# mikelodder7/bls-bn254

Hardware: AMD Instinct MI355X
Metric: BN254 pairings/sec (= BLS verifies/sec) (higher is better)
Workload: dtype int64; 1 GPU; 262144 batched single-sig BLS verifies per GPU (BASELINE configs[1]), unique 32-byte messages, 1024-key pool, 1/64 invalid tuples; key de-duplication + hash-to-G1 + per-key G2 checks and line tables + 2-pair Miller loop + final exp; tuples_per_gpu=262144, tuples_total=262144, key_pool=1024

## Files before the change

### bls-bn254_amd/csrc/host.hip

```cpp
#include "host_common.h"

extern "C" {

const uint8_t NEG_G2_BYTES[128] = {
  0x19,0x8e,0x93,0x93,0x92,0x0d,0x48,0x3a,0x72,0x60,0xbf,0xb7,0x31,0xfb,0x5d,0x25,0xf1,0xaa,0x49,0x33,0x35,0xa9,0xe7,0x12,0x97,0xe4,0x85,0xb7,0xae,0xf3,0x12,0xc2,
  0x18,0x00,0xde,0xef,0x12,0x1f,0x1e,0x76,0x42,0x6a,0x00,0x66,0x5e,0x5c,0x44,0x79,0x67,0x43,0x22,0xd4,0xf7,0x5e,0xda,0xdd,0x46,0xde,0xbd,0x5c,0xd9,0x92,0xf6,0xed,
  0x27,0x5d,0xc4,0xa2,0x88,0xd1,0xaf,0xb3,0xcb,0xb1,0xac,0x09,0x18,0x75,0x24,0xc7,0xdb,0x36,0x39,0x5d,0xf7,0xbe,0x3b,0x99,0xe6,0x73,0xb1,0x3a,0x07,0x5a,0x65,0xec,
  0x1d,0x9b,0xef,0xcd,0x05,0xa5,0x32,0x3e,0x6d,0xa4,0xd4,0x35,0xf3,0xb6,0x17,0xcd,0xb3,0xaf,0x83,0x28,0x5c,0x2d,0xf7,0x11,0xef,0x39,0xc0,0x15,0x71,0x82,0x7f,0x9d};


const char* blsbn254_strerror(int code) {
  switch (code) {
    case 0: return "ok";
    case 1: return "invalid scalar bytes";
    case 2: return "invalid G1 bytes";
    case 3: return "invalid G2 bytes";
    case 4: return "invalid Gt bytes";
    case BLSBN254_ST_SHORT: return "too few usable partial signatures";
    case BLSBN254_E_ARG: return "invalid argument";
    case BLSBN254_E_HIP: return "HIP runtime error";
    case BLSBN254_E_NOMEM: return "out of device memory";
    case BLSBN254_E_NO_DEVICE: return "no gfx950 device available (there is no CPU fallback)";
    case BLSBN254_E_RCCL: return "RCCL error";
    default: return "unknown error";
  }
}
const char* blsbn254_last_error(blsbn254_ctx* ctx) { return ctx ? ctx->last_error.c_str() : ""; }

int blsbn254_ctx_create(int device, blsbn254_ctx** out) {
  if (!out) return BLSBN254_E_ARG;
  *out = nullptr;
  int count = 0;
  if (hipGetDeviceCount(&count) != hipSuccess || count <= 0 || device < 0 || device >= count) return BLSBN254_E_NO_DEVICE;
  hipDeviceProp_t prop;
  if (hipGetDeviceProperties(&prop, device) != hipSuccess) return BLSBN254_E_NO_DEVICE;
  if (std::strncmp(prop.gcnArchName, "gfx950", 6) != 0) return BLSBN254_E_NO_DEVICE;
  blsbn254_ctx* c = new blsbn254_ctx();
  c->device = device;
  if (const char* e = std::getenv("BLSBN254_CHUNK_LANES")) {
    size_t v = (size_t)std::strtoull(e, nullptr, 10) & ~(size_t)7;
    if (v >= 8 && v <= ((size_t)1 << 23)) c->chunk = v;
  }
  if (hipSetDevice(device) != hipSuccess || hipStreamCreateWithFlags(&c->stream, hipStreamNonBlocking) != hipSuccess) { delete c; return BLSBN254_E_HIP; }
  if (hipStreamCreateWithFlags(&c->stream2, hipStreamNonBlocking) != hipSuccess || hipEventCreateWithFlags(&c->ev_fork, hipEventDisableTiming) != hipSuccess ||
      hipEventCreateWithFlags(&c->ev_join, hipEventDisableTiming) != hipSuccess) { (void)hipStreamDestroy(c->stream); delete c; return BLSBN254_E_HIP; }
  if (getrandom(&c->kd_seed, sizeof c->kd_seed, 0) != (ssize_t)sizeof c->kd_seed) c->kd_seed = 0x5bd1e995u;
  if (const char* e = std::getenv("BLSBN254_AUTO_PREPARE")) c->auto_prepare = std::atoi(e) != 0;
  if (const char* e = std::getenv("BLSBN254_RLC_GROUP")) { long v = std::atol(e); if (v >= 2 && v <= 4096) { c->rlc_group = (size_t)v; c->rlc_group_auto = false; } }
  c->lanes_per_round = (size_t)prop.multiProcessorCount * 256;
  if (const char* e = std::getenv("BLSBN254_RLC_KEY_ROUND")) c->rlc_key_round = std::atoi(e) != 0;
  if (const char* e = std::getenv("BLSBN254_WIDE_FE")) c->wide_fe = std::atoi(e) != 0;
  if (const char* e = std::getenv("BLSBN254_ASYNC_VERIFY")) c->async_verify = std::atoi(e) != 0;
  if (const char* e = std::getenv("BLSBN254_KEY_CACHE")) { long v = std::atol(e); if (v >= 0 && v <= (long)PREP_MAX_KEYS) c->kc.max = (size_t)v; }
  if (const char* e = std::getenv("BLSBN254_QUAD_PREP")) c->quad_prep = std::atoi(e) != 0;
  if (const char* e = std::getenv("BLSBN254_SPLIT_EASY")) c->split_easy = std::atoi(e) != 0;
  c->tri_max = c->lanes_per_round / 4;
  if (const char* e = std::getenv("BLSBN254_TRI_MILLER")) c->tri_miller = std::atoi(e) != 0;
  if (const char* e = std::getenv("BLSBN254_TRI_FE")) c->tri_fe = std::atoi(e) != 0;
  if (const char* e = std::getenv("BLSBN254_TRI_MAX")) { long v = std::atol(e); if (v >= 0 && v <= (1 << 20)) c->tri_max = (size_t)v; }
  if (const char* e = std::getenv("BLSBN254_WIDE_FE_MAX")) { long v = std::atol(e); if (v >= 0 && v <= (1 << 20)) c->wide_fe_max = (size_t)v; }
  *out = c;
  return 0;
}
void blsbn254_ctx_destroy(blsbn254_ctx* c) {
  if (!c) return;
  (void)hipSetDevice(c->device);
  (void)hipStreamSynchronize(c->stream);
  (void)hipStreamSynchronize(c->stream2);
  for (auto& pv : c->pend) if (pv.ev) (void)hipEventDestroy(pv.ev);
  if (c->pend_host) (void)hipHostFree(c->pend_host);
  for (auto& kv : c->prof) for (auto& pr : kv.second.pending) { (void)hipEventDestroy(pr.first); (void)hipEventDestroy(pr.second); }
  (void)hipEventDestroy(c->ev_fork); (void)hipEventDestroy(c->ev_join);
  (void)hipStreamDestroy(c->stream2);
  (void)hipStreamDestroy(c->stream);
  delete c;
}
int blsbn254_ctx_synchronize(blsbn254_ctx* c) {
  if (!c) return BLSBN254_E_ARG;
  ENTER(c);
  HIPCHK(c, hipStreamSynchronize(c->stream));
  return 0;
}
void* blsbn254_ctx_stream(blsbn254_ctx* c) { return c ? (void*)c->stream : nullptr; }

int blsbn254_profile_enable(blsbn254_ctx* c, int on) { if (!c) return BLSBN254_E_ARG; c->profiling = on != 0; return 0; }
int blsbn254_profile_reset(blsbn254_ctx* c) {
  if (!c) return BLSBN254_E_ARG;
  HIPCHK(c, hipStreamSynchronize(c->stream));
  for (auto& kv : c->prof) for (auto& pr : kv.second.pending) { (void)hipEventDestroy(pr.first); (void)hipEventDestroy(pr.second); }
  c->prof.clear();
  return 0;
}
int blsbn254_profile_read(blsbn254_ctx* c, char* names, uint64_t* launches, double* total_ms, int max_entries) {
  if (!c) return BLSBN254_E_ARG;
  HIPCHK(c, hipStreamSynchronize(c->stream));
  int k = 0;
  for (auto& kv : c->prof) {
    ProfEntry& p = kv.second;
    for (auto& pr : p.pending) { float ms = 0; (void)hipEventElapsedTime(&ms, pr.first, pr.second); p.ms += ms; (void)hipEventDestroy(pr.first); (void)hipEventDestroy(pr.second); }
    p.pending.clear();
    if (k < max_entries) { std::snprintf(names + 32 * k, 32, "%s", kv.first.c_str()); launches[k] = p.launches; total_ms[k] = p.ms; ++k; }
  }
  return k;
}

struct EventPair {
  hipEvent_t e0 = nullptr, e1 = nullptr;
  ~EventPair() { if (e0) (void)hipEventDestroy(e0); if (e1) (void)hipEventDestroy(e1); }
// ... 43 lines not shown
  return 0;
}

int stage_dst(blsbn254_ctx* c, const uint8_t* dst, size_t dst_len, uint32_t* out_len) {
  uint8_t tmp[256];
  if (dst_len > 255) {
    Sha256 s; sha256_init(s);
    sha256_update(s, (const uint8_t*)"H2C-OVERSIZE-DST-", 17); sha256_update(s, dst, dst_len); sha256_final(s, tmp);
    dst_len = 32;
  } else if (dst_len) std::memcpy(tmp, dst, dst_len);
  *out_len = (uint32_t)dst_len;
  if (c->dst_host_len == (int)dst_len && (dst_len == 0 || std::memcmp(c->dst_host, tmp, dst_len) == 0)) return 0;
  HIPCHK(c, c->dst.reserve(256));
  c->dst_host_len = -1;
  if (dst_len) {
    HIPCHK(c, hipStreamSynchronize(c->stream));
    std::memcpy(c->dst_host, tmp, dst_len);
    HIPCHK(c, hipMemcpyAsync(c->dst.p, c->dst_host, dst_len, hipMemcpyHostToDevice, c->stream));
  }
  c->dst_host_len = (int)dst_len;
  return 0;
}
int check_offsets(const uint64_t* off, size_t n) {
  for (size_t i = 0; i < n; ++i) if (off[i + 1] < off[i]) return BLSBN254_E_ARG;
  return 0;
}
int min_index_arm(blsbn254_ctx* c, int* d, size_t words) {
  static const int none[2] = {NO_INDEX, NO_INDEX};
  HIPCHK(c, hipMemcpyAsync(d, none, 4 * words, hipMemcpyHostToDevice, c->stream));
  return 0;
}
int min_index_read(blsbn254_ctx* c, const int* d, int* out) {
  TRY(download(c, out, d, 4));
  if (*out == NO_INDEX) *out = -1;
  return 0;
}
int first_bad(blsbn254_ctx* c, const uint8_t* d_status, size_t n, uint8_t mask, uint8_t val, int* out) {
  HIPCHK(c, c->misc.reserve(64));
  TRY(min_index_arm(c, (int*)c->misc.p, 1));
  TRY(launch(c, c->stream, "status_reduce", grid_lanes(n), k_status_reduce, d_status, n, mask, val, (int*)c->misc.p));
  return min_index_read(c, (const int*)c->misc.p, out);
}
int read_status(blsbn254_ctx* c, const uint8_t* d_status, int idx, uint8_t* st) { return download(c, st, d_status + idx, 1); }


int run_final_exp(blsbn254_ctx* c, int32_t* f, size_t n, size_t stride, int mode, const uint8_t* flags, const uint8_t* sub_ok,
                         uint8_t* d_bitmap, uint8_t* d_gt, int* d_is_one) {
  CHECK_LANES(c, stride);
  for (DevBuf& b : c->fe) HIPCHK(c, b.reserve(stride * 108 * 4));
  HIPCHK(c, c->fe_slots.reserve(stride * 108 * 4 * 10));
  int32_t* S = (int32_t*)c->fe_slots.p;
  int32_t *X = (int32_t*)c->fe[0].p, *A = (int32_t*)c->fe[1].p, *B = (int32_t*)c->fe[2].p, *C = (int32_t*)c->fe[3].p,
          *B2 = (int32_t*)c->fe[4].p, *D = (int32_t*)c->fe[5].p;
  if (n >= c->lanes_per_round / 2 && c->split_easy) {
    TRY(launch(c, c->stream, "fe_easy_head", grid_lanes(n), k_fe_easy_head, (const int32_t*)f, n, stride, A, B));
    TRY(launch(c, c->stream, "fe_inv4", grid_lanes((n + 3) / 4), k_fe_inv4, B, n, stride));
    TRY(launch(c, c->stream, "fe_easy_tail", grid_lanes(n), k_fe_easy_tail, (const int32_t*)f, f, n, stride, (const int32_t*)A, (const int32_t*)B));
  } else {
    TRY(launch(c, c->stream, "fe_easy", grid_lanes(n), k_fe_easy, (const int32_t*)f, f, n, stride));
  }
  if (c->wide_fe && n <= c->wide_fe_max) {
    uint8_t* one = nullptr;
    if (mode == 0) { HIPCHK(c, c->fe_wide_one.reserve(n)); one = (uint8_t*)c->fe_wide_one.p; }
    TRY(launch(c, c->stream, "fe_hard_wide", grid_wide(n), k_fe_hard_wide, (const int32_t*)f, n, stride, flags, sub_ok, one, d_gt, d_is_one, mode));
    if (mode == 0) TRY(launch(c, c->stream, "pack_bitmap", grid_lanes(n), k_pack_bitmap, (const uint8_t*)one, n, d_bitmap));
    return 0;
  }
  if (n <= c->tri_max && c->tri_fe) {
    HIPCHK(c, c->tri_vals.reserve(n * TRI_VALUE_LIMBS * 4));
    uint8_t* one = nullptr;
    if (mode == 0) { HIPCHK(c, c->fe_wide_one.reserve(n)); one = (uint8_t*)c->fe_wide_one.p; }
    TRY(launch(c, c->stream, "fe_tri_hard", grid_tri(n), k_fe_tri_hard, (const int32_t*)f, n, stride, (int32_t*)c->tri_vals.p, flags, sub_ok, one, d_gt, d_is_one, mode));
    if (mode == 0) TRY(launch(c, c->stream, "pack_bitmap", grid_lanes(n), k_pack_bitmap, (const uint8_t*)one, n, d_bitmap));
    return 0;
  }
  TRY(launch(c, c->stream, "fe_expx_h1", grid_lanes(n), k_fe_expx_h1, (const int32_t*)f, S, n, stride, A, B));
  TRY(launch(c, c->stream, "fe_expx_h2", grid_lanes(n), k_fe_expx_h2, (const int32_t*)B, S, n, stride, B, C, B2, D));
  TRY(launch(c, c->stream, "fe_expx", grid_lanes(n), k_fe_expx, (const int32_t*)D, X, S, n, stride));
  TRY(launch(c, c->stream, "fe_h3", grid_lanes(n), k_fe_h3, (const int32_t*)f, (const int32_t*)A, (const int32_t*)C, (const int32_t*)B2, (const int32_t*)X, S, n, stride,
             flags, sub_ok, d_bitmap, d_gt, d_is_one, mode));
  return 0;
}

int miller_to_ws(blsbn254_ctx* c, const uint8_t* d_g1, const uint8_t* d_g2, size_t n) {
  CHECK_LANES(c, n);
  HIPCHK(c, c->f_ws.reserve(n * 108 * 4));
  HIPCHK(c, c->status.reserve(n));
  if (c->wide_fe && n <= c->wide_fe_max / 2) {
    TRY(launch(c, c->stream, "miller_wide_1", grid_wide(n), k_miller_wide_1, d_g1, d_g2, n, (int32_t*)c->f_ws.p, n, (uint8_t*)c->status.p));
  } else if (n <= c->tri_max && c->tri_miller) {
    TRY(launch(c, c->stream, "miller_tri_1", grid_tri(n), k_miller_tri_1, d_g1, d_g2, n, (int32_t*)c->f_ws.p, n, (uint8_t*)c->status.p));
  } else {
    TRY(launch(c, c->stream, "miller_1", grid_lanes(n), k_miller_1, d_g1, d_g2, n, (int32_t*)c->f_ws.p, n, (uint8_t*)c->status.p));
  }
  return 0;
}
int decode_status_rc(blsbn254_ctx* c, const uint8_t* d_status, size_t n) {
  int bad;
  int rc = first_bad(c, d_status, n, 3, 3, &bad);
  if (rc) return rc;
  if (bad < 0) return 0;
  uint8_t st; rc = read_status(c, d_status, bad, &st);
  if (rc) return rc;
  return (st & 1) ? BLSBN254_ERR_G2 : BLSBN254_ERR_G1;
}
int blsbn254_pairing_batch_dev(blsbn254_ctx* c, const uint8_t* d_g1, const uint8_t* d_g2, size_t n, uint8_t* d_gt, uint8_t* d_status) {
  if (!c || (n && (!d_g1 || !d_g2 || !d_gt))) return BLSBN254_E_ARG;
// ... 126 lines not shown
```

### bls-bn254_amd/csrc/host_common.h

```cpp
#pragma once
#include <hip/hip_runtime.h>
#include <sys/random.h>
#include <cstdio>
#include <cstdlib>
#include <cstring>
#include <algorithm>
#include <map>
#include <string>
#include <vector>

#include "sha256.h"
#include "lane_ops.h"
#include "kernels.h"
#include "key_cache.h"
#include "seg_plan.h"
#include "keyset_agg_plan.h"
#include "keyset_merge_plan.h"
#include "keyset_weight_plan.h"
#include "keyset_committee_plan.h"
#include "keyset_rlc_plan.h"
#include "../../include/blsbn254.h"

using namespace bn;

// ... 90 lines not shown
  DevBuf keys, table, valid, slots, state, slot_of, miss_rep, miss_slot, tslot, cslot, batch_ok;
  size_t max = 4096;
  size_t cap = 0;
  uint32_t mask = 0;
};
struct ProfEntry { uint64_t launches = 0; std::vector<std::pair<hipEvent_t, hipEvent_t>> pending; double ms = 0; };

struct blsbn254_ctx {
  int device = 0;
  hipStream_t stream = nullptr;
  DevBuf in_a, in_b, in_c, in_off, dst, h_ws, f_ws, f_ws2, flags, sub_ok, status, bitmap, out, scalars, misc;
  DevBuf fe[6];
  DevBuf rlc_a2, rlc_a, rlc_b, rlc_elig, rlc_f2, rlc_bytes, rlc_neg, rlc_ok, rlc_idx, rlc_cpk, rlc_csig, rlc_ch, rlc_csub, rlc_cbm;
  DevBuf r2_seed, r2_a, r2_b, r2_sigok, r2_tchunk, r2_ccnt, r2_cbase, r2_ckid, r2_cstart, r2_clen, r2_csig, r2_ch, r2_cstate, r2_iota, r2_cisone,
         r2_need, r2_bcnt, r2_bbase, r2_list, r2_valid;
  DevBuf ks_cnt[2], ks_base[2], ks_kid[2], ks_start, ks_len, ks_tchunk, ks_iota, ks_out[2], ks_out2[2];
  DevBuf r2_sa, r2_sb, r2_celig, r2_kelig, r2_ksig, r2_kh, r2_kstate, r2_kisone, r2_kpass, r2_cpass, r2_clist, r2_cneed, r2_cbcnt, r2_cbbase;
  bool rlc_key_round = true;
  unsigned rlc_key_skip = 0, rlc_key_streak = 0;
  size_t rlc_group = 16;
  bool rlc_group_auto = true;
  size_t lanes_per_round = 65536;
  uint64_t stat_rlc_key_rounds = 0, stat_rlc_key_rounds_passed = 0;
  uint64_t stat_rlc[4] = {0, 0, 0, 0};
  DevBuf status_all;
  DevBuf kd_slots, kd_rep, kd_kid, kd_keys, kd_hist, kd_cursor, kd_perm, kd_cnt, prep_table, prep_raw, prep_ok, prep_isone, prep_valid;
  KeyStore kc;
  hipStream_t stream2 = nullptr;
  hipEvent_t ev_fork = nullptr, ev_join = nullptr;
  bool s2_pending = false;
  uint32_t kd_seed = 0;
  bool auto_prepare = true;
  uint64_t stat_prepared_chunks = 0, stat_exact_chunks = 0, stat_grouped_aggregates = 0, stat_pairwise_aggregates = 0;
  DevBuf q_ws;
  DevBuf th_x, th_num, th_den, th_glv, th_part, th_part2;
  DevBuf fe_wide_one;
  bool wide_fe = true;
  size_t tri_max = 16384;
  bool tri_miller = true, tri_fe = true;
  DevBuf tri_vals;
  struct PendingVerify {
    bool active = false; const uint8_t *d_pks = nullptr, *d_msgs = nullptr, *d_sigs = nullptr; const uint64_t* d_off = nullptr;
    size_t n = 0; uint8_t* d_bitmap = nullptr; uint8_t dst[256]; size_t dst_len = 0; hipEvent_t ev = nullptr;
  } pend[4];
  int pend_head = 0, pend_count = 0;
  uint32_t* pend_host = nullptr;
  DevBuf pend_dev;
  size_t u_hint = 0;
  size_t u_max_seen = 0;
  bool async_verify = true;
  uint64_t stat_async_chunks = 0, stat_async_reruns = 0;
  bool quad_prep = true;
  bool split_easy = true;
  size_t wide_fe_max = 2048;
  DevBuf gs_items, gs_items_ok, gs_sum, gs_sum_ok, gs_pk;
  SegWs gs;
  DevBuf fe_slots;
  uint8_t dst_host[256];
  int dst_host_len = -1;
  size_t chunk = (size_t)1 << 22;
  MsmWs msm;
  PcWs pc;
  ThbWs thb;
  AgbWs agb;
  TdlWs tdl;
  TcWs tc;
  KsetWs kset;
  KaggWs kagg;
  KmWs kmrg;
  KwWs kw;
  KcWs kcom;
  KsrWs ksr;
  uint64_t stat_kset[4] = {0, 0, 0, 0};
  uint64_t stat_kw[4] = {0, 0, 0, 0};
  uint64_t stat_kc[4] = {0, 0, 0, 0};
  size_t ksr_group = KSR_DEFAULT_GROUP;
  uint64_t stat_ksr[6] = {0, 0, 0, 0, 0, 0};
  uint64_t stat_kagg[4] = {0, 0, 0, 0};
  uint64_t stat_kmrg[4] = {0, 0, 0, 0};
  uint64_t stat_tc[4] = {0, 0, 0, 0};
  uint64_t stat_tdl[4] = {0, 0, 0, 0};
  uint64_t stat_agb[4] = {0, 0, 0, 0};
  uint64_t stat_thb[3] = {0, 0, 0};
  int msm_window = 0;
  uint64_t stat_msm[4] = {0, 0, 0, 0};
  bool profiling = false;
  std::map<std::string, ProfEntry> prof;
  std::string last_error;
};

#define HIPCHK(ctx, x) do { hipError_t e_ = (x); if (e_ != hipSuccess) { (ctx)->last_error = std::string(#x) + ": " + hipGetErrorString(e_); \
    return e_ == hipErrorOutOfMemory ? BLSBN254_E_NOMEM : BLSBN254_E_HIP; } } while (0)

#define TRY(x) do { int rc_ = (x); if (rc_) return rc_; } while (0)

static inline unsigned nblocks(size_t n) { return (unsigned)((n + 255) / 256); }
struct Shape { dim3 grid, block; };
static inline Shape grid_lanes(size_t n) { return {dim3(nblocks(n)), dim3(256)}; }
static inline Shape grid_tri(size_t n) { return {dim3((unsigned)((n + 63) / 64)), dim3(256)}; }
static inline Shape grid_wide(size_t n) { return {dim3((unsigned)n), dim3(128)}; }
static const size_t TRI_VALUE_LIMBS = 20 * 108;

struct BNH ProfScope {
  blsbn254_ctx* c; hipStream_t s; const char* name; hipEvent_t e0 = nullptr, e1 = nullptr;
  ProfScope(blsbn254_ctx* c_, hipStream_t s_, const char* n) : c(c_), s(s_), name(c_->profiling ? n : nullptr) {
    if (name) { (void)hipEventCreate(&e0); (void)hipEventCreate(&e1); (void)hipEventRecord(e0, s); }
// ... 158 lines not shown
```

### bls-bn254_amd/csrc/k_fe_easy.hip

```cpp
#include "lane_ops.h"
#include "kernels.h"
using namespace bn;

BN_KERNEL k_fe_easy(const int32_t* in, int32_t* out, size_t n, size_t stride) {
  size_t i = (size_t)blockIdx.x * blockDim.x + threadIdx.x;
  if (i >= n) return;
  fp12_store_limbs(out + i, stride, fe_easy(fp12_load_limbs(in + i, stride)));
}
BN_KERNEL k_fe_easy_head(const int32_t* in, size_t n, size_t stride, int32_t* head, int32_t* nu) {
  size_t i = (size_t)blockIdx.x * blockDim.x + threadIdx.x;
  if (i >= n) return;
  const FeEasyHead h = fe_easy_head(fp12_load_limbs(in + i, stride));
  fp2_store_limbs(head + i, stride, h.c0); fp2_store_limbs(head + 18 * stride + i, stride, h.c1);
  fp2_store_limbs(head + 36 * stride + i, stride, h.c2); fp2_store_limbs(head + 54 * stride + i, stride, h.nrm);
  store_fp(nu + i, stride, h.nu);
}
BN_KERNEL k_fe_inv4(int32_t* nu, size_t n, size_t stride) {
  const size_t q = (n + 3) / 4;
  size_t j = (size_t)blockIdx.x * blockDim.x + threadIdx.x;
  if (j >= q) return;
  Fp x[4];
  for (int t = 0; t < 4; ++t) { const size_t i = j + (size_t)t * q; x[t] = i < n ? load_fp(nu + i, stride) : fp_one(); }
  fp_inv4(x);
  for (int t = 0; t < 4; ++t) { const size_t i = j + (size_t)t * q; if (i < n) store_fp(nu + i, stride, x[t]); }
}
```

### bls-bn254_amd/csrc/k_fe_easy_tail.hip

```cpp
#include "lane_ops.h"
#include "kernels.h"
using namespace bn;

BN_KERNEL k_fe_easy_tail(const int32_t* in, int32_t* out, size_t n, size_t stride, const int32_t* head, const int32_t* nu) {
  size_t i = (size_t)blockIdx.x * blockDim.x + threadIdx.x;
  if (i >= n) return;
  FeEasyHead h;
  h.c0 = fp2_load_limbs(head + i, stride); h.c1 = fp2_load_limbs(head + 18 * stride + i, stride);
  h.c2 = fp2_load_limbs(head + 36 * stride + i, stride); h.nrm = fp2_load_limbs(head + 54 * stride + i, stride);
  h.nu = fp_zero();
  fp12_store_limbs(out + i, stride, fe_easy_tail(fp12_load_limbs(in + i, stride), h, load_fp(nu + i, stride)));
}
```

### bls-bn254_amd/csrc/k_fe_expx.hip

```cpp
#include "lane_ops.h"
#include "kernels.h"
using namespace bn;

BN_KERNEL k_fe_expx(const int32_t* in, int32_t* out, int32_t* slots, size_t n, size_t stride) {
  __shared__ int32_t park_lds[108 * 256];
  size_t i = (size_t)blockIdx.x * blockDim.x + threadIdx.x;
  if (i >= n) return;
  const Ws park = {park_lds, 256, threadIdx.x * 4u, false};
  fp12_store_limbs(out + i, stride, cyclotomic_exp_x_chain(fp12_load_limbs(in + i, stride), Ws{slots, stride, (uint32_t)i * 4u, true}, &park));
}
```

### bls-bn254_amd/csrc/k_fe_expx_tail.hip

```cpp
#include "lane_ops.h"
#include "kernels.h"
using namespace bn;

BN_KERNEL k_fe_expx_h1(const int32_t* in, int32_t* slots, size_t n, size_t stride, int32_t* a_out, int32_t* b_out) {
  __shared__ int32_t park_lds[108 * 256];
  size_t i = (size_t)blockIdx.x * blockDim.x + threadIdx.x;
  if (i >= n) return;
  const uint32_t l4 = (uint32_t)i * 4u;
  const Ws park = {park_lds, 256, threadIdx.x * 4u, false};
  Fp12 r = cyclotomic_exp_x_chain(fp12_load_limbs(in + i, stride), Ws{slots, stride, l4, true}, &park);
  fe_h1_tail(r, Ws{a_out, stride, l4, true}, Ws{b_out, stride, l4, true}, &park);
}
BN_KERNEL k_fe_expx_h2(const int32_t* in, int32_t* slots, size_t n, size_t stride, int32_t* b_in, int32_t* c_out, int32_t* b2_out, int32_t* d2_out) {
  __shared__ int32_t park_lds[108 * 256];
  size_t i = (size_t)blockIdx.x * blockDim.x + threadIdx.x;
  if (i >= n) return;
  const uint32_t l4 = (uint32_t)i * 4u;
  const Ws park = {park_lds, 256, threadIdx.x * 4u, false};
  Fp12 r = cyclotomic_exp_x_chain(fp12_load_limbs(in + i, stride), Ws{slots, stride, l4, true}, &park);
  fe_h2_tail(r, Ws{b_in, stride, l4, true}, Ws{c_out, stride, l4, true}, Ws{b2_out, stride, l4, true}, Ws{d2_out, stride, l4, true}, &park);
}
```

### bls-bn254_amd/csrc/pairing.h

```cpp
#pragma once
#include "curve.h"

namespace bn {

struct G2J { Fp2 x, y, z; };
struct Line { Fp2 c0, c1, c2; };

BN_FUNC Line doubling_step(G2J& r) {
  BN_CTX;
  Fp2 tmp0 = fp2_sqr(r.x);
  Fp2 tmp1 = fp2_sqr(r.y);
  Fp2 tmp2 = fp2_sqr(tmp1);
  Fp2 s3 = fp2_sqr(fp2_norm(fp2_add(tmp1, r.x)));
  Fp2 tmp3 = f_lc3<2, -2, -2>(s3, tmp0, tmp2);
  Fp2 tmp4 = f_lc2<3, 0>(tmp0, tmp0);
  Fp2 tmp6 = fp2_norm(fp2_add(r.x, tmp4));
  Fp2 tmp5 = fp2_sqr(tmp4);
  Fp2 zsq = fp2_sqr(r.z);
  Fp2 nx = f_lc2<1, -2>(tmp5, tmp3);
  Fp2 nz = fp2_norm(fp2_sub(fp2_sub(fp2_sqr(fp2_norm(fp2_add(r.z, r.y))), tmp1), zsq));
  Fp2 ny = f_lc2<1, -8>(fp2_mul(fp2_sub(tmp3, nx), tmp4), tmp2);
  Line l;
  l.c1 = f_lc2<-2, 0>(fp2_mul(tmp4, zsq), zsq);
  Fp2 s6 = fp2_sub(fp2_sub(fp2_sqr(tmp6), tmp0), tmp5);
// ... 290 lines not shown
  f = miller2_step<3>(f, T, park, lpark, hh, qw, false, live_a, live_b);
  return f;
}

BN_FUNC Fp12 cyclotomic_exp_x(const Fp12& f) {
  BN_CTX;
  Fp12 r = f;
  for (int i = 61; i >= 0; --i) {
    r = fp12_cyclotomic_sqr(r);
    if ((bnc::BN_X >> i) & 1) r = fp12_mul(r, f);
  }
  return r;
}
BN_FUNC Fp12 cyclotomic_exp_x_chain(const Fp12& f, const Ws& slots, const Ws* park = nullptr) {
  const ChainOp prog[BN_X_CHAIN_LEN] = BN_X_CHAIN;
  fp12_store_mem(slots, f);
  BN_MEM_FENCE;
  Fp12 r = f;
  for (int k = 0; k < BN_X_CHAIN_LEN; ++k) {
    const ChainOp op = prog[k];
    if (op.load >= 0) r = fp12_load_mem(ws_at(slots, 108 * op.load));
    for (int q = 0; q < op.sq; ++q) r = fp12_cyclotomic_sqr(r);
    if (op.mul >= 0) r = fp12_mul_mem(r, ws_at(slots, 108 * op.mul), park);
    if (op.store >= 0) fp12_store_mem(ws_at(slots, 108 * op.store), r);
    if (op.cstore >= 0) { fp6_store_mem(ws_at(slots, 108 * op.cstore), r.c0); fp6_store_mem(ws_at(slots, 108 * op.cstore + 54), fp6_norm(fp6_neg(r.c1))); }
    if (op.store >= 0 || op.cstore >= 0) BN_MEM_FENCE;
  }
  return r;
}
BN_FUNC Fp12 fe_easy(const Fp12& f) {
  Fp12 t = fp12_mul(fp12_conj(f), fp12_inv(f));
  return fp12_mul(fp12_frob<2>(t), t);
}
struct FeEasyHead { Fp2 c0, c1, c2, nrm; Fp nu; };
BN_FUNC FeEasyHead fe_easy_head(const Fp12& a) {
  BN_CTX;
  Fp6 s0 = fp6_sqr(a.c0), s1 = fp6_sqr(a.c1);
  Fp6 d = {fp2_sub_mul_xi(s0.c0, s1.c2), fp2_norm(fp2_sub(s0.c1, s1.c0)), fp2_norm(fp2_sub(s0.c2, s1.c1))};
  Fp2 q0 = fp2_sqr(d.c0), q1 = fp2_sqr(d.c1), q2 = fp2_sqr(d.c2);
  Fp2 m01 = fp2_mul(d.c0, d.c1), m02 = fp2_mul(d.c0, d.c2), m12 = fp2_mul(d.c1, d.c2);
  FeEasyHead h;
  h.c0 = fp2_sub_mul_xi(q0, m12);
  h.c1 = fp2_norm(fp2_sub(fp2_mul_xi(q2), m01));
  h.c2 = fp2_norm(fp2_sub(q1, m02));
  Fp2 u = fp2_add(fp2_mul(d.c2, h.c1), fp2_mul(d.c1, h.c2));
  h.nrm = fp2_add_mul_xi(fp2_mul(d.c0, h.c0), u);
  h.nu = fp_dot2(h.nrm.c0, h.nrm.c0, h.nrm.c1, h.nrm.c1);
  return h;
}
BN_FUNC Fp12 fe_easy_tail(const Fp12& a, const FeEasyHead& h, const Fp& nu_inv) {
  BN_CTX;
  Fp2 ti = {fp_mul(h.nrm.c0, nu_inv), fp_mul(fp_neg(h.nrm.c1), nu_inv)};
  Fp6 t6 = {fp2_mul(h.c0, ti), fp2_mul(h.c1, ti), fp2_mul(h.c2, ti)};
  Fp12 inv = {fp6_mul(a.c0, t6), fp6_norm(fp6_neg(fp6_mul(a.c1, t6)))};
  Fp12 t = fp12_mul(fp12_conj(a), inv);
  return fp12_mul(fp12_frob<2>(t), t);
}
template <bool POW_FALLBACK = true>
BN_FUNC bool fp_inv4(Fp x[4]) {
  BN_CTX;
  bool z[4];
  Fp v[4], pre[4];
  for (int i = 0; i < 4; ++i) { z[i] = fp_is_zero(x[i]); v[i] = fp_select(z[i], fp_one(), fp_norm(x[i])); }
  pre[0] = v[0];
  for (int i = 1; i < 4; ++i) pre[i] = fp_mul(pre[i - 1], v[i]);
  bool done = true;
  Fp inv = POW_FALLBACK ? fp_inv(pre[3]) : fp_inv_divsteps(pre[3], done);
  for (int i = 3; i >= 1; --i) {
    Fp r = fp_mul(inv, pre[i - 1]);
    inv = fp_mul(inv, v[i]);
    x[i] = fp_select(z[i], fp_zero(), r);
  }
  x[0] = fp_select(z[0], fp_zero(), inv);
  return done;
}
BN_FUNC void fe_h1(const Fp12& x0, Fp12& a, Fp12& b) {
  a = fp12_cyclotomic_sqr(fp12_conj(x0));
  Fp12 a2 = fp12_cyclotomic_sqr(a);
  b = fp12_mul(a, a2);
}
BN_FUNC void fe_h2(const Fp12& x0, const Fp12& b, Fp12& c, Fp12& b2, Fp12& d2) {
  c = fp12_conj(x0);
  b2 = fp12_mul(c, fp12_conj(b));
  d2 = fp12_cyclotomic_sqr(c);
}
BN_FUNC Fp12 fe_h3(const Fp12& t, const Fp12& a, const Fp12& c, const Fp12& b2, const Fp12& x0) {
  Fp12 e = fp12_mul(b2, x0);
  Fp12 d = fp12_mul(a, e);
  Fp12 l0 = fp12_mul(t, fp12_mul(c, e));
  Fp12 r = fp12_mul(l0, fp12_frob<1>(d));
  r = fp12_mul(r, fp12_frob<2>(e));
  Fp12 l3 = fp12_mul(fp12_conj(t), d);
  return fp12_mul(r, fp12_frob<3>(l3));
}
BN_FUNC Fp12 final_exponentiation(const Fp12& f) {
  Fp12 t = fe_easy(f), a, b, c, b2, d2;
  fe_h1(cyclotomic_exp_x(t), a, b);
  fe_h2(cyclotomic_exp_x(b), b, c, b2, d2);
  return fe_h3(t, a, c, b2, cyclotomic_exp_x(d2));
}

BN_INL void fp2_to_be(uint8_t* out, const Fp2& c) { fp_to_be(out, c.c0); fp_to_be(out + 32, c.c1); }
BN_FUNC void fp12_to_be(uint8_t* out, const Fp12& a) {
  BN_CTX;
  fp2_to_be(out, a.c0.c0); fp2_to_be(out + 64, a.c0.c1); fp2_to_be(out + 128, a.c0.c2);
  fp2_to_be(out + 192, a.c1.c0); fp2_to_be(out + 256, a.c1.c1); fp2_to_be(out + 320, a.c1.c2);
}
BN_INL Fp2 fp2_from_be(const uint8_t* in, bool& ok) {
// ... 86 lines not shown
}

BN_FUNC void fe_h1_tail(const Fp12& x0, const Ws& a_out, const Ws& b_out, const Ws* park) {
  Fp12 a = fp12_cyclotomic_sqr(fp12_conj(x0));
  fp12_store_mem(a_out, a);
  BN_MEM_FENCE;
  fp12_store_mem(b_out, fp12_mul_mem(fp12_cyclotomic_sqr(a), a_out, park));
}
BN_FUNC void fe_h2_tail(const Fp12& x0, const Ws& b_in, const Ws& c_out, const Ws& b2_out, const Ws& d2_out, const Ws* park) {
  fp12_store_mem(c_out, fp12_conj(x0));
  BN_MEM_FENCE;
  fp12_store_mem(b2_out, fp12_conj(fp12_mul_mem(x0, b_in, park)));
  BN_MEM_FENCE;
  fp12_store_mem(d2_out, fp12_cyclotomic_sqr(fp12_load_mem(c_out)));
}

BN_INL void line_store_limbs(const Ws& w, const Line& l) { fp2_store_limbs(w, l.c0); fp2_store_limbs(ws_at(w, 18), l.c1); fp2_store_limbs(ws_at(w, 36), l.c2); }
BN_INL Line line_load_limbs(const Ws& w) { return {fp2_load_limbs(w), fp2_load_limbs(ws_at(w, 18)), fp2_load_limbs(ws_at(w, 36))}; }
BN_FUNC void g2_prepare_lines(const G2A& q, const Ws& out) {
  BN_CTX;
  G2J T = {q.x, q.y, fp2_one()};
  Fp2 nqy = fp2_norm(fp2_neg(q.y));
  int ti = 0;
  for (int j = bnc::ATE_NAF_LEN - 2; j >= 0; --j) {
    line_store_limbs(ws_at(out, 54 * (size_t)ti++), doubling_step(T));
    int d = ate_naf_digit(j);
    if (d != 0) line_store_limbs(ws_at(out, 54 * (size_t)ti++), addition_step(T, q.x, d > 0 ? q.y : nqy));
  }
  Fp2 g2 = fp2_const(bnc::GAMMA1[1]), g3 = fp2_const(bnc::GAMMA1[2]);
  Fp2 q1x = fp2_mul(fp2_norm(fp2_conj(q.x)), g2), q1y = fp2_mul(fp2_norm(fp2_conj(q.y)), g3);
  Fp2 q2x = fp2_mul(fp2_norm(fp2_conj(q1x)), g2);
  Fp2 q2y = fp2_norm(fp2_neg(fp2_mul(fp2_norm(fp2_conj(q1y)), g3)));
  line_store_limbs(ws_at(out, 54 * (size_t)ti++), addition_step(T, q1x, q1y));
  line_store_limbs(ws_at(out, 54 * (size_t)ti++), addition_step(T, q2x, q2y));
}
BN_INL void fp_store_limbs_lazy(const Ws& w, const Fp& c) {
  BN_TRK(if (c.lo < -4e-6 || c.hi > 1.0 + 4e-6 || c.tlo < -0.02 || c.thi > 0.02 || c.vb > 1.2) check_fail("pair table entry outside its declared range", c.vb);)
  BN_UNROLL for (int k = 0; k < NL; ++k) ws_store(w, k, c.l[k]);
}
BN_INL Fp fp_load_limbs_lazy(const Ws& w) {
  Fp c;
  BN_UNROLL for (int k = 0; k < NL; ++k) c.l[k] = ws_load(w, k);
  BN_TRK(set_trk(c, -4e-6, 1.0 + 4e-6, -0.02, 0.02, 1.2); check_actual(c, "pair table entry");)
  return c;
}
BN_INL void fp2_store_limbs_lazy(const Ws& w, const Fp2& c) { fp_store_limbs_lazy(w, c.c0); fp_store_limbs_lazy(ws_at(w, 9), c.c1); }
BN_INL Fp2 fp2_load_limbs_lazy(const Ws& w) {
  Fp2 c;
  BN_UNROLL for (int k = 0; k < NL; ++k) { c.c0.l[k] = ws_load(w, k); c.c1.l[k] = ws_load(w, 9 + k); }
  BN_TRK(set_trk(c.c0, -4e-6, 1.0 + 4e-6, -0.02, 0.02, 1.2); set_trk(c.c1, -4e-6, 1.0 + 4e-6, -0.02, 0.02, 1.2);
         check_actual(c.c0, "pair table entry"); check_actual(c.c1, "pair table entry");)
  return c;
}
BN_FUNC void line_pair_expand(const Line& a, const Line& b, const Ws& out) {
  BN_CTX;
  fp2_store_limbs_lazy(out, fp2_mul(a.c0, b.c0));
  fp2_store_limbs_lazy(ws_at(out, 18), fp2_mul_xi(fp2_mul(a.c2, b.c2)));
  fp2_store_limbs_lazy(ws_at(out, 36), fp2_mul(a.c1, b.c1));
  fp2_store_limbs_lazy(ws_at(out, 54), fp2_mul(a.c1, b.c2));
  fp2_store_limbs_lazy(ws_at(out, 72), fp2_mul(a.c2, b.c1));
  fp2_store_limbs_lazy(ws_at(out, 90), fp2_mul(a.c0, b.c1));
  fp2_store_limbs_lazy(ws_at(out, 108), fp2_mul(a.c1, b.c0));
  fp2_store_limbs_lazy(ws_at(out, 126), fp2_mul(a.c0, b.c2));
  fp2_store_limbs_lazy(ws_at(out, 144), fp2_mul(a.c2, b.c0));
}
BN_INL Fp2 fp2_dot_fp(const Fp2& t, const Fp& s, const Fp2& u, const Fp& r) {
  return {fp_dot2(t.c0, s, u.c0, r), fp_dot2(t.c1, s, u.c1, r)};
}
BN_FUNC Fp12 ell_pair_expanded(const Fp12& f, const Ws& e, const Ws& cw) {
  BN_CTX;
  Fp X = fp_load_mem(cw), Y = fp_load_mem(ws_at(cw, 9)), Z = fp_load_mem(ws_at(cw, 18));
  Fp xsX = fp_load_mem(ws_at(cw, 27)), ysY = fp_load_mem(ws_at(cw, 36)), xsZ = fp_load_mem(ws_at(cw, 45));
  Fp ysZ = fp_load_mem(ws_at(cw, 54)), ysX = fp_load_mem(ws_at(cw, 63)), xsY = fp_load_mem(ws_at(cw, 72));
  Fp6 l0 = {fp2_dot_fp(fp2_load_limbs_lazy(e), ysY, fp2_load_limbs_lazy(ws_at(e, 18)), Z),
            fp2_mul_fp(fp2_load_limbs_lazy(ws_at(e, 36)), xsX),
            fp2_dot_fp(fp2_load_limbs_lazy(ws_at(e, 54)), xsZ, fp2_load_limbs_lazy(ws_at(e, 72)), X)};
  Fp2 l10 = fp2_dot_fp(fp2_load_limbs_lazy(ws_at(e, 90)), ysX, fp2_load_limbs_lazy(ws_at(e, 108)), xsY);
  Fp2 l11 = fp2_dot_fp(fp2_load_limbs_lazy(ws_at(e, 126)), ysZ, fp2_load_limbs_lazy(ws_at(e, 144)), Y);
  Fp6 v0 = fp6_mul(f.c0, l0);
  Fp6 v1 = fp6_mul_by_01(f.c1, l10, l11);
  Fp6 dl = {fp2_norm(fp2_sub(l10, l0.c0)), fp2_norm(fp2_sub(l11, l0.c1)), fp2_norm(fp2_neg(l0.c2))};
  Fp6 w = fp6_mul(fp6_norm(fp6_sub(f.c0, f.c1)), dl);
  return {fp6_add_mul_v(v0, v1), fp6_norm(fp6_add(fp6_add(w, v0), v1))};
}
BN_FUNC Fp12 miller_loop_prepared(const Ws& inv, const Ws& ktab_in) {
  Fp12 f = fp12_one();
  Ws p = inv, kt = ktab_in;
  int ti = 0;
  for (int j = bnc::ATE_NAF_LEN - 2; j >= 0; --j) {
    f = fp12_sqr(f);
    BN_OPAQUE(kt); BN_OPAQUE(p);
    f = ell_pair_expanded(f, ws_at(kt, 162 * (size_t)ti), p);
    ++ti;
    if (ate_naf_digit(j) != 0) {
      BN_OPAQUE(kt); BN_OPAQUE(p);
      f = ell_pair_expanded(f, ws_at(kt, 162 * (size_t)ti), p);
      ++ti;
    }
  }
  for (int e = 0; e < 2; ++e) {
    BN_OPAQUE(kt); BN_OPAQUE(p);
    f = ell_pair_expanded(f, ws_at(kt, 162 * (size_t)ti), p);
    ++ti;
  }
  return f;
}
// ... 165 lines not shown
```

Before: 8.088 million verifies/s.

## Use lazy Fp12 loads/stores across final-exp kernels and cheaper easy-part tail

```diff
diff --git a/bls-bn254_amd/csrc/host.hip b/bls-bn254_amd/csrc/host.hip
--- a/bls-bn254_amd/csrc/host.hip
+++ b/bls-bn254_amd/csrc/host.hip
@@ -54,6 +54,8 @@
   if (const char* e = std::getenv("BLSBN254_KEY_CACHE")) { long v = std::atol(e); if (v >= 0 && v <= (long)PREP_MAX_KEYS) c->kc.max = (size_t)v; }
   if (const char* e = std::getenv("BLSBN254_QUAD_PREP")) c->quad_prep = std::atoi(e) != 0;
   if (const char* e = std::getenv("BLSBN254_SPLIT_EASY")) c->split_easy = std::atoi(e) != 0;
+  c->split_easy_min = c->lanes_per_round / 2;
+  if (const char* e = std::getenv("BLSBN254_SPLIT_EASY_MIN")) { long v = std::atol(e); if (v >= 1 && v <= (1 << 20)) c->split_easy_min = (size_t)v; }
   c->tri_max = c->lanes_per_round / 4;
   if (const char* e = std::getenv("BLSBN254_TRI_MILLER")) c->tri_miller = std::atoi(e) != 0;
   if (const char* e = std::getenv("BLSBN254_TRI_FE")) c->tri_fe = std::atoi(e) != 0;
@@ -203,7 +205,8 @@
   int32_t* S = (int32_t*)c->fe_slots.p;
   int32_t *X = (int32_t*)c->fe[0].p, *A = (int32_t*)c->fe[1].p, *B = (int32_t*)c->fe[2].p, *C = (int32_t*)c->fe[3].p,
           *B2 = (int32_t*)c->fe[4].p, *D = (int32_t*)c->fe[5].p;
-  if (n >= c->lanes_per_round / 2 && c->split_easy) {
+  const bool lane_hard = !(c->wide_fe && n <= c->wide_fe_max) && !(n <= c->tri_max && c->tri_fe);
+  if (n >= c->split_easy_min && c->split_easy && lane_hard) {
     TRY(launch(c, c->stream, "fe_easy_head", grid_lanes(n), k_fe_easy_head, (const int32_t*)f, n, stride, A, B));
     TRY(launch(c, c->stream, "fe_inv4", grid_lanes((n + 3) / 4), k_fe_inv4, B, n, stride));
     TRY(launch(c, c->stream, "fe_easy_tail", grid_lanes(n), k_fe_easy_tail, (const int32_t*)f, f, n, stride, (const int32_t*)A, (const int32_t*)B));
diff --git a/bls-bn254_amd/csrc/host_common.h b/bls-bn254_amd/csrc/host_common.h
--- a/bls-bn254_amd/csrc/host_common.h
+++ b/bls-bn254_amd/csrc/host_common.h
@@ -166,6 +166,7 @@
   uint64_t stat_async_chunks = 0, stat_async_reruns = 0;
   bool quad_prep = true;
   bool split_easy = true;
+  size_t split_easy_min = 32768;
   size_t wide_fe_max = 2048;
   DevBuf gs_items, gs_items_ok, gs_sum, gs_sum_ok, gs_pk;
   SegWs gs;
diff --git a/bls-bn254_amd/csrc/k_fe_easy.hip b/bls-bn254_amd/csrc/k_fe_easy.hip
--- a/bls-bn254_amd/csrc/k_fe_easy.hip
+++ b/bls-bn254_amd/csrc/k_fe_easy.hip
@@ -5,12 +5,12 @@
 BN_KERNEL k_fe_easy(const int32_t* in, int32_t* out, size_t n, size_t stride) {
   size_t i = (size_t)blockIdx.x * blockDim.x + threadIdx.x;
   if (i >= n) return;
-  fp12_store_limbs(out + i, stride, fe_easy(fp12_load_limbs(in + i, stride)));
+  fp12_store_limbs(out + i, stride, fe_easy(fp12_load_limbs_lazy(in + i, stride)));
 }
 BN_KERNEL k_fe_easy_head(const int32_t* in, size_t n, size_t stride, int32_t* head, int32_t* nu) {
   size_t i = (size_t)blockIdx.x * blockDim.x + threadIdx.x;
   if (i >= n) return;
-  const FeEasyHead h = fe_easy_head(fp12_load_limbs(in + i, stride));
+  const FeEasyHead h = fe_easy_head(fp12_load_limbs_lazy(in + i, stride));
   fp2_store_limbs(head + i, stride, h.c0); fp2_store_limbs(head + 18 * stride + i, stride, h.c1);
   fp2_store_limbs(head + 36 * stride + i, stride, h.c2); fp2_store_limbs(head + 54 * stride + i, stride, h.nrm);
   store_fp(nu + i, stride, h.nu);
diff --git a/bls-bn254_amd/csrc/k_fe_easy_tail.hip b/bls-bn254_amd/csrc/k_fe_easy_tail.hip
--- a/bls-bn254_amd/csrc/k_fe_easy_tail.hip
+++ b/bls-bn254_amd/csrc/k_fe_easy_tail.hip
@@ -9,5 +9,5 @@
   h.c0 = fp2_load_limbs(head + i, stride); h.c1 = fp2_load_limbs(head + 18 * stride + i, stride);
   h.c2 = fp2_load_limbs(head + 36 * stride + i, stride); h.nrm = fp2_load_limbs(head + 54 * stride + i, stride);
   h.nu = fp_zero();
-  fp12_store_limbs(out + i, stride, fe_easy_tail(fp12_load_limbs(in + i, stride), h, load_fp(nu + i, stride)));
+  fp12_store_limbs_lazy(out + i, stride, fe_easy_tail(fp12_load_limbs_lazy(in + i, stride), h, load_fp(nu + i, stride)));
 }
diff --git a/bls-bn254_amd/csrc/k_fe_expx.hip b/bls-bn254_amd/csrc/k_fe_expx.hip
--- a/bls-bn254_amd/csrc/k_fe_expx.hip
+++ b/bls-bn254_amd/csrc/k_fe_expx.hip
@@ -7,5 +7,5 @@
   size_t i = (size_t)blockIdx.x * blockDim.x + threadIdx.x;
   if (i >= n) return;
   const Ws park = {park_lds, 256, threadIdx.x * 4u, false};
-  fp12_store_limbs(out + i, stride, cyclotomic_exp_x_chain(fp12_load_limbs(in + i, stride), Ws{slots, stride, (uint32_t)i * 4u, true}, &park));
+  fp12_store_limbs(out + i, stride, cyclotomic_exp_x_chain(fp12_load_limbs_lazy(in + i, stride), Ws{slots, stride, (uint32_t)i * 4u, true}, &park));
 }
diff --git a/bls-bn254_amd/csrc/k_fe_expx_tail.hip b/bls-bn254_amd/csrc/k_fe_expx_tail.hip
--- a/bls-bn254_amd/csrc/k_fe_expx_tail.hip
+++ b/bls-bn254_amd/csrc/k_fe_expx_tail.hip
@@ -8,7 +8,7 @@
   if (i >= n) return;
   const uint32_t l4 = (uint32_t)i * 4u;
   const Ws park = {park_lds, 256, threadIdx.x * 4u, false};
-  Fp12 r = cyclotomic_exp_x_chain(fp12_load_limbs(in + i, stride), Ws{slots, stride, l4, true}, &park);
+  Fp12 r = cyclotomic_exp_x_chain(fp12_load_limbs_lazy(in + i, stride), Ws{slots, stride, l4, true}, &park);
   fe_h1_tail(r, Ws{a_out, stride, l4, true}, Ws{b_out, stride, l4, true}, &park);
 }
 BN_KERNEL k_fe_expx_h2(const int32_t* in, int32_t* slots, size_t n, size_t stride, int32_t* b_in, int32_t* c_out, int32_t* b2_out, int32_t* d2_out) {
@@ -17,6 +17,6 @@
   if (i >= n) return;
   const uint32_t l4 = (uint32_t)i * 4u;
   const Ws park = {park_lds, 256, threadIdx.x * 4u, false};
-  Fp12 r = cyclotomic_exp_x_chain(fp12_load_limbs(in + i, stride), Ws{slots, stride, l4, true}, &park);
+  Fp12 r = cyclotomic_exp_x_chain(fp12_load_limbs_lazy(in + i, stride), Ws{slots, stride, l4, true}, &park);
   fe_h2_tail(r, Ws{b_in, stride, l4, true}, Ws{c_out, stride, l4, true}, Ws{b2_out, stride, l4, true}, Ws{d2_out, stride, l4, true}, &park);
 }
diff --git a/bls-bn254_amd/csrc/pairing.h b/bls-bn254_amd/csrc/pairing.h
--- a/bls-bn254_amd/csrc/pairing.h
+++ b/bls-bn254_amd/csrc/pairing.h
@@ -366,8 +366,13 @@
   BN_CTX;
   Fp2 ti = {fp_mul(h.nrm.c0, nu_inv), fp_mul(fp_neg(h.nrm.c1), nu_inv)};
   Fp6 t6 = {fp2_mul(h.c0, ti), fp2_mul(h.c1, ti), fp2_mul(h.c2, ti)};
+#ifdef BN_EASY_TAIL_DENSE
   Fp12 inv = {fp6_mul(a.c0, t6), fp6_norm(fp6_neg(fp6_mul(a.c1, t6)))};
   Fp12 t = fp12_mul(fp12_conj(a), inv);
+#else
+  Fp12 s = fp12_sqr(fp12_conj(a));
+  Fp12 t = {fp6_mul(s.c0, t6), fp6_mul(s.c1, t6)};
+#endif
   return fp12_mul(fp12_frob<2>(t), t);
 }
 template <bool POW_FALLBACK = true>
@@ -560,6 +565,38 @@
          check_actual(c.c0, "pair table entry"); check_actual(c.c1, "pair table entry");)
   return c;
 }
+constexpr int WS_LAZY_VB = 8, WS_LAZY_VB_VVW = 16;
+#ifdef BN_CHECK
+inline void ws_lazy_check(const Fp& c, double vb) {
+  const double top = vb * P_OVER_R + 1e-6;
+  if (c.lo < -4e-6 || c.hi > 1.0 + 4e-6 || c.tlo < -top || c.thi > top || c.vb > vb) check_fail("inter-phase value outside its declared range", c.vb);
+}
+inline void ws_lazy_declare(Fp& c, double vb) { set_trk(c, -4e-6, 1.0 + 4e-6, -(vb * P_OVER_R + 1e-6), vb * P_OVER_R + 1e-6, vb); check_actual(c, "inter-phase value"); }
+#endif
+template <int VB>
+BN_INL void fp2_ws_store_lazy(const Ws& w, int at, const Fp2& c) {
+  BN_TRK(ws_lazy_check(c.c0, VB); ws_lazy_check(c.c1, VB);)
+  BN_UNROLL for (int k = 0; k < NL; ++k) { ws_store(w, at + k, c.c0.l[k]); ws_store(w, at + 9 + k, c.c1.l[k]); }
+}
+template <int VB>
+BN_INL Fp2 fp2_ws_load_lazy(const Ws& w, int at) {
+  Fp2 c;
+  BN_UNROLL for (int k = 0; k < NL; ++k) { c.c0.l[k] = ws_load(w, at + k); c.c1.l[k] = ws_load(w, at + 9 + k); }
+  BN_TRK(ws_lazy_declare(c.c0, VB); ws_lazy_declare(c.c1, VB);)
+  return c;
+}
+BN_FUNC void fp12_store_limbs_lazy(const Ws& w, const Fp12& a) {
+  BN_CTX;
+  fp2_ws_store_lazy<WS_LAZY_VB>(w, 0, a.c0.c0); fp2_ws_store_lazy<WS_LAZY_VB>(w, 18, a.c0.c1); fp2_ws_store_lazy<WS_LAZY_VB>(w, 36, a.c0.c2);
+  fp2_ws_store_lazy<WS_LAZY_VB>(w, 54, a.c1.c0); fp2_ws_store_lazy<WS_LAZY_VB>(w, 72, a.c1.c1); fp2_ws_store_lazy<WS_LAZY_VB_VVW>(w, 90, a.c1.c2);
+}
+BN_FUNC Fp12 fp12_load_limbs_lazy(const Ws& w) {
+  BN_CTX;
+  return {{fp2_ws_load_lazy<WS_LAZY_VB>(w, 0), fp2_ws_load_lazy<WS_LAZY_VB>(w, 18), fp2_ws_load_lazy<WS_LAZY_VB>(w, 36)},
+          {fp2_ws_load_lazy<WS_LAZY_VB>(w, 54), fp2_ws_load_lazy<WS_LAZY_VB>(w, 72), fp2_ws_load_lazy<WS_LAZY_VB_VVW>(w, 90)}};
+}
+BN_FUNC void fp12_store_limbs_lazy(int32_t* out, size_t stride, const Fp12& a) { fp12_store_limbs_lazy(Ws{out, stride, 0, false}, a); }
+BN_FUNC Fp12 fp12_load_limbs_lazy(const int32_t* in, size_t stride) { return fp12_load_limbs_lazy(Ws{const_cast<int32_t*>(in), stride, 0, false}); }
 BN_FUNC void line_pair_expand(const Line& a, const Line& b, const Ws& out) {
   BN_CTX;
   fp2_store_limbs_lazy(out, fp2_mul(a.c0, b.c0));
```

New measurement: 8.128 million verifies/s, median of 6. No clear change (+0.5%).
